# vikramarsid/cadence

Measured on AMD Instinct MI355X. Metric: history events replayed/sec + workflows rebuilt/sec (node), % of HBM roofline, higher is better.
Workload: dtype int64

## Files before the change

### cadence_amd/csrc/replay.hip

```cpp
#include <hip/hip_runtime.h>

#include <cstdio>
#include <cstdlib>
#include <cstring>
#include <type_traits>
#include <vector>

#include "cdr/cdr.h"
#include "ctx.h"

#ifndef CDR_DEPTH
#define CDR_DEPTH 1
#endif
#ifndef CDR_TYPED
#define CDR_TYPED 1
#endif
#ifndef CDR_WPE
#define CDR_WPE 3
#endif
#ifndef CDR_LDS_ACT_MAX
#define CDR_LDS_ACT_MAX 1
#endif
#ifndef CDR_LDS_TIM_MAX
#define CDR_LDS_TIM_MAX 4
// ... 2235 lines not shown
    if (reg0 && carry) {
      launch_reg<CDR_REG0_NA, CDR_REG0_NT, CDR_REG0_NX, CDR_SLICE_REG0, 3, true>(tasks, gr0, sx(3), out_list(Lr0, 3, 1));
      carry_tail(3, gr0, sx(3), true);
    } else if (reg0) {
      typedef RegLds<CDR_REG0_NA, CDR_REG0_NT, CDR_REG0_NX> LY;
      if (cls) {
        typedef ClsLds<CDR_REG0_NA, CDR_REG0_NT, CDR_REG0_NX> LC;
        if (tasks)
          hipLaunchKernelGGL((k_replay_cls<CDR_REG0_NA, CDR_REG0_NT, CDR_REG0_NX, CDR_SLICE_REG0, CDR_WPE_CLS_T, false, true>),
                             gr0, dim3(CDR_SLICE_WIDTH), LC::bytes + CLS_TQ_BYTES, sx(3), with_list(Lr0, 3));
        else
          hipLaunchKernelGGL((k_replay_cls<CDR_REG0_NA, CDR_REG0_NT, CDR_REG0_NX, CDR_SLICE_REG0, CDR_WPE_CLS0>), gr0,
                             dim3(CDR_SLICE_WIDTH), LC::bytes, sx(3), with_list(Lr0, 3));
      }
      if (cls && tasks)
        hipLaunchKernelGGL(k_tasks_merge<CDR_SLICE_REG0>, gr0, dim3(CDR_SLICE_WIDTH), 9 * 65 * 8, sx(3), Lr0);
      if (tasks && !cls)
        hipLaunchKernelGGL((k_replay_reg<CDR_REG0_NA, CDR_REG0_NT, CDR_REG0_NX, CDR_SLICE_REG0, CDR_WPE_REG, false, true>), gr0,
                           dim3(CDR_SLICE_WIDTH), LY::bytes, sx(3), Lr0);
      else if (!cls)
        hipLaunchKernelGGL((k_replay_reg<CDR_REG0_NA, CDR_REG0_NT, CDR_REG0_NX, CDR_SLICE_REG0, 3>), gr0, dim3(CDR_SLICE_WIDTH), LY::bytes, sx(3),
                           Lr0);
    }
        break;
      case 4:
    if (fst && tasks) hipLaunchKernelGGL(k_replay_fast<true>, gf, dim3(CDR_SLICE_WIDTH), FAST_LDS_BYTES + FAST_TBUF_BYTES, sx(4), Lf);
    else if (fst) hipLaunchKernelGGL(k_replay_fast<false>, gf, dim3(CDR_SLICE_WIDTH), FAST_LDS_BYTES, sx(4), Lf);
        break;
      case 5:
    if (reg1 && carry) {
      launch_reg<CDR_REG_NA, CDR_REG_NT, CDR_REG_NX, CDR_SLICE_REG, CDR_WPE_REG, true>(tasks, gr1, sx(5), out_list(Lr1, 5, 1));
      carry_tail(5, gr1, sx(5), true);
    } else if (reg1) {
      typedef RegLds<CDR_REG_NA, CDR_REG_NT, CDR_REG_NX> LY;
      if (cls) {
        typedef ClsLds<CDR_REG_NA, CDR_REG_NT, CDR_REG_NX> LC;
        if (tasks)
          hipLaunchKernelGGL((k_replay_cls<CDR_REG_NA, CDR_REG_NT, CDR_REG_NX, CDR_SLICE_REG, CDR_WPE_CLS_T, false, true>),
                             gr1, dim3(CDR_SLICE_WIDTH), LC::bytes + CLS_TQ_BYTES, sx(5), with_list(Lr1, 5));
        else
          hipLaunchKernelGGL((k_replay_cls<CDR_REG_NA, CDR_REG_NT, CDR_REG_NX, CDR_SLICE_REG, CDR_WPE_CLS>), gr1,
                             dim3(CDR_SLICE_WIDTH), LC::bytes, sx(5), with_list(Lr1, 5));
      }
      if (cls && tasks)
        hipLaunchKernelGGL(k_tasks_merge<CDR_SLICE_REG>, gr1, dim3(CDR_SLICE_WIDTH), 9 * 65 * 8, sx(5), Lr1);
      if (tasks && !cls)
        hipLaunchKernelGGL((k_replay_reg<CDR_REG_NA, CDR_REG_NT, CDR_REG_NX, CDR_SLICE_REG, CDR_WPE_REG, false, true>), gr1,
                           dim3(CDR_SLICE_WIDTH), LY::bytes, sx(5), Lr1);
      else if (!cls)
        hipLaunchKernelGGL((k_replay_reg<CDR_REG_NA, CDR_REG_NT, CDR_REG_NX, CDR_SLICE_REG>), gr1, dim3(CDR_SLICE_WIDTH), LY::bytes, sx(5),
                           Lr1);
    }
        break;
    }
  };
  auto launch_retry = [&](int i) {
    if (!cls || !cls_fb || carry) return;
    switch (i) {
      case 6:
        if (par && !tasks) {
          typedef RegLds<CDR_REG2_NA, CDR_REG_NT, CDR_REG_NX> LY;
          cdr_launch Lp = L;
          Lp.s0 = 0;
          hipLaunchKernelGGL((k_replay_reg<CDR_REG2_NA, CDR_REG_NT, CDR_REG_NX, CDR_SLICE_PAR>), retry_grid(dim3(npar)),
                             dim3(CDR_SLICE_WIDTH), LY::bytes, st, retry_of(with_list(Lp, 6)));
        }
        break;
      case 1:
        if (reg2) {
          typedef RegLds<CDR_REG2_NA, CDR_REG_NT, CDR_REG_NX> LY;
          if (tasks)
            hipLaunchKernelGGL((k_replay_reg<CDR_REG2_NA, CDR_REG_NT, CDR_REG_NX, CDR_SLICE_REG2, CDR_WPE_REG, false, true>),
                               retry_grid(gr2), dim3(CDR_SLICE_WIDTH), LY::bytes, st, retry_of(with_list(Lr2, 1)));
          else
            hipLaunchKernelGGL((k_replay_reg<CDR_REG2_NA, CDR_REG_NT, CDR_REG_NX, CDR_SLICE_REG2>), retry_grid(gr2),
                               dim3(CDR_SLICE_WIDTH), LY::bytes, st, retry_of(with_list(Lr2, 1)));
        }
        break;
      case 3:
        if (reg0) {
          typedef RegLds<CDR_REG0_NA, CDR_REG0_NT, CDR_REG0_NX> LY;
          if (tasks)
            hipLaunchKernelGGL((k_replay_reg<CDR_REG0_NA, CDR_REG0_NT, CDR_REG0_NX, CDR_SLICE_REG0, CDR_WPE_REG, false, true>),
                               retry_grid(gr0), dim3(CDR_SLICE_WIDTH), LY::bytes, st, retry_of(with_list(Lr0, 3)));
          else
            hipLaunchKernelGGL((k_replay_reg<CDR_REG0_NA, CDR_REG0_NT, CDR_REG0_NX, CDR_SLICE_REG0, 3>), retry_grid(gr0),
                               dim3(CDR_SLICE_WIDTH), LY::bytes, st, retry_of(with_list(Lr0, 3)));
        }
        break;
      case 5:
        if (reg1) {
          typedef RegLds<CDR_REG_NA, CDR_REG_NT, CDR_REG_NX> LY;
          if (tasks)
            hipLaunchKernelGGL((k_replay_reg<CDR_REG_NA, CDR_REG_NT, CDR_REG_NX, CDR_SLICE_REG, CDR_WPE_REG, false, true>),
                               retry_grid(gr1), dim3(CDR_SLICE_WIDTH), LY::bytes, st, retry_of(with_list(Lr1, 5)));
          else
            hipLaunchKernelGGL((k_replay_reg<CDR_REG_NA, CDR_REG_NT, CDR_REG_NX, CDR_SLICE_REG>), retry_grid(gr1),
                               dim3(CDR_SLICE_WIDTH), LY::bytes, st, retry_of(with_list(Lr1, 5)));
        }
        break;
    }
  };
  bool issued[cdr_ctx::N_SIDE] = {};
  if (gating) {
    for (int j = 0; j < cdr_ctx::N_SIDE; j++) {
      const int i = order[j] - '0';
      if ((gate && i == 6) || (gate2 && i == 1)) {
        launch_class(i);
        HIPCHK(hipGetLastError());
        issued[i] = true;
      }
    }
    hipStream_t waited[cdr_ctx::N_SIDE + 1];
    int nw = 0;
    for (int q = 0; q < 6; q++) {
      if (!on[q] || q == 1 || (gate && sx(q) == sx(6)) || (gate2 && sx(q) == sx(1))) continue;
      bool dup = false;
      for (int r = 0; r < nw; r++) dup |= waited[r] == sx(q);
      if (dup) continue;
      waited[nw++] = sx(q);
      HIPCHK(hipStreamWaitValue32(sx(q), rws + 15, gate_n, hipStreamWaitValueGte, 0xFFFFFFFFu));
    }
  }
  for (int j = 0; j < cdr_ctx::N_SIDE; j++) {
    const int i = order[j] - '0';
    if (issued[i]) continue;
    launch_class(i);
    HIPCHK(hipGetLastError());
  }
  for (int j = 0; j < cdr_ctx::N_SIDE; j++)
    if (used[j]) {
      HIPCHK(hipEventRecord(c->join[j], c->side[j]));
      HIPCHK(hipStreamWaitEvent(st, c->join[j], 0));
    }
  for (int i : {6, 1, 3, 5}) launch_retry(i);
  HIPCHK(hipGetLastError());
  HIPCHK(hipEventRecord(ring ? c->ring[c->ring_used + 1] : c->ev[1], st));
  if (ring) {
    c->ring_used += 2;
    HIPCHK(hipEventRecord(c->ev[0], st));
    HIPCHK(hipEventRecord(c->ev[1], st));
  }
  const uint32_t fb = (in->n_wfs + 255) / 256;
  const bool all_fast = fst && kinds == 1 && in->n_fast_slices == blocks && gf.x == blocks && !carry && !rws;
  if (fb && !all_fast) hipLaunchKernelGGL(k_tables, dim3(fb), dim3(256), 0, st, *in, *out);
  HIPCHK(hipGetLastError());
  if (fb) hipLaunchKernelGGL(k_finalize, dim3(fb), dim3(256), 0, st, *in, *out);
  HIPCHK(hipGetLastError());
  HIPCHK(hipEventRecord(c->ev[2], st));
  c->timed = true;
  return CDR_API_OK;
}

uint32_t cdr_build_flags(void) {
  uint32_t f = 0;
#ifdef CDR_PAR_PROF
  f |= 1u;
#endif
  if (CDR_PAR_PRIO != 0 || CDR_FDEPTH != 2 || CDR_DEPTH != 1 || CDR_TYPED != 1 || CDR_FAST_DELTA != 1 || CDR_FAST_HINT != 1 ||
      CDR_VHBF != 1 || CDR_VHQUICK != 1 || CDR_CLS_DEPTH != 1 || CDR_CLS_PDEPTH != 4 || CDR_CLS_DEPTH_PAR != 4 ||
      CDR_CLS_PDEPTH_PAR != 16 || CDR_WPE_FAST != 3 || CDR_WPE != 3 || CDR_WPE_CLS != 4 || CDR_WPE_CLS0 != 4 ||
      CDR_WPE_CLS2 != 2 || FAST_CK != 8u || CDR_FAST_TBUF != 5 || CDR_WPE_FAST_TBUF != 2)
    f |= 2u;
  return f;
}

int cdr_last_kernel_ms(cdr_ctx* c, float* replay_ms, float* finalize_ms) {
  if (!c || !c->timed) return CDR_API_EINVAL;
  HIPCHK(hipEventSynchronize(c->ev[2]));
  float a = 0, b = 0;
  HIPCHK(hipEventElapsedTime(&a, c->ev[0], c->ev[1]));
  HIPCHK(hipEventElapsedTime(&b, c->ev[1], c->ev[2]));
  if (replay_ms) *replay_ms = a;
  if (finalize_ms) *finalize_ms = b;
  return CDR_API_OK;
}

int cdr_timing_begin(cdr_ctx* c, uint32_t max_launches) {
  if (!c) return CDR_API_EINVAL;
  HIPCHK(hipSetDevice(c->device));
  while (c->ring.size() < 2ull * max_launches) {
    hipEvent_t e;
    HIPCHK(hipEventCreate(&e));
    c->ring.push_back(e);
  }
  c->ring_used = 0;
  return CDR_API_OK;
}

int cdr_timing_read(cdr_ctx* c, float* ms, uint32_t* n) {
  if (!c || !n) return CDR_API_EINVAL;
  const uint32_t k = c->ring_used / 2;
  for (uint32_t i = 0; i < k && i < *n; i++) {
    HIPCHK(hipEventSynchronize(c->ring[2 * i + 1]));
    HIPCHK(hipEventElapsedTime(&ms[i], c->ring[2 * i], c->ring[2 * i + 1]));
  }
  *n = k < *n ? k : *n;
  c->ring_used = (uint32_t)c->ring.size();
  return CDR_API_OK;
}

}
```

### cadence_amd/csrc/replay_fast.inc

```
#ifndef CDR_WPE_FAST
#define CDR_WPE_FAST 3
#endif
#ifndef CDR_FDEPTH
#define CDR_FDEPTH 2
#endif
constexpr uint32_t FD = CDR_FDEPTH;
#ifndef CDR_VHBF
#define CDR_VHBF 1
#endif
#ifndef CDR_VHQUICK
#define CDR_VHQUICK 1
#endif
#ifndef CDR_FAST_TBUF
#define CDR_FAST_TBUF 5
#endif
#ifndef CDR_TQ_NT
#define CDR_TQ_NT 1
#endif
#ifndef CDR_WPE_FAST_TBUF
#define CDR_WPE_FAST_TBUF 2
#endif
#ifndef CDR_FAST_SADDR
#define CDR_FAST_SADDR 1
#endif
#ifndef CDR_FAST_QROW
#define CDR_FAST_QROW 1
#endif
#ifndef CDR_FAST_DELTA
#define CDR_FAST_DELTA 1
#endif
#ifndef CDR_FAST_HINT
#define CDR_FAST_HINT 1
#endif
#define FAST_LOAD_OPS load_ops<CDR_FAST_DELTA, CDR_NT_FAST, CDR_FAST_HINT != 0>
__device__ __forceinline__ int64_t mov64(int64_t x) {
  int64_t y;
  asm volatile("v_mov_b64 %0, %1" : "=v"(y) : "v"(x));
  return y;
}
__device__ __forceinline__ uint32_t mov32(uint32_t x) {
  uint32_t y;
  asm volatile("v_mov_b32 %0, %1" : "=v"(y) : "v"(x));
  return y;
}
__device__ __forceinline__ uint32_t tf_take(uint32_t t) { return mov32(t); }
__device__ __forceinline__ Ev ev_take(const Ev& q) {
  Ev e;
  e.tf = mov32(q.tf);
  e.h = mov32(q.h);
  e.n = (int32_t)mov32((uint32_t)q.n);
  e.id = mov64(q.id);
  e.ver = mov64(q.ver);
  e.ts = mov64(q.ts);
  e.key = mov64(q.key);
  e.aux = mov64(q.aux);
  return e;
}
#ifndef FAST_CK
#define FAST_CK 8u
#endif
enum : uint32_t {
  ZP_DST_TS = 0, ZP_DSC_TS, ZP_DORIG_TS, ZP_LAST_PROCESSED, ZP_COMPLETION_BATCH,
  ZP_VH_OFF, ZP_RP_OFF, ZP_RUN_RPCAP, ZP_CK0, FAST_COLD = ZP_CK0 + FAST_CK / 2
};
template <class O>
__device__ __forceinline__ GAS cdr_vh_item* fast_out_vh(const O& o) { return gp(o.vh); }
template <class O>
__device__ __forceinline__ GAS cdr_reset_point* fast_out_rp(const O& o) { return gp(o.rp); }
#define VM_DRAIN() __builtin_amdgcn_s_waitcnt(0x0F70)
#define FAST_LDS_BYTES ((CDR_ACT_PLANES + FAST_COLD) * CDR_SLICE_WIDTH * sizeof(uint64_t))
#define FAST_TQ_WORDS (3u * CDR_FAST_TBUF * CDR_SLICE_WIDTH)
#define FAST_TBUF_BYTES (FAST_TQ_WORDS * sizeof(uint64_t))

template <bool TASKS = false>
__global__ __launch_bounds__(CDR_SLICE_WIDTH) __attribute__((amdgpu_waves_per_eu(TASKS && CDR_FAST_TBUF > 0 ? CDR_WPE_FAST_TBUF : CDR_WPE_FAST, 8))) void
k_replay_fast(cdr_launch L) {
  (void)L;
  const uint32_t s = blockIdx.x + KA()->s0;
  const uint32_t lane = threadIdx.x;
  if (s >= KA()->B.ev.n_slices || !KA()->fast) return;
  const uint32_t sflags = __builtin_amdgcn_readfirstlane(KA()->B.ev.slice_flags[s]);
  if (!(sflags & CDR_SLICE_FAST)) return;
  const uint64_t row0_ = KA()->B.ev.slice_row0[s];
  const uint64_t row0 = ((uint64_t)__builtin_amdgcn_readfirstlane((uint32_t)(row0_ >> 32)) << 32) |
                        __builtin_amdgcn_readfirstlane((uint32_t)row0_);
  Slice S;
  S.elems = __builtin_amdgcn_readfirstlane(KA()->B.ev.slice_len[s]) * CDR_SLICE_WIDTH;
  S.r = __builtin_amdgcn_make_buffer_rsrc((void*)(KA()->B.ev.slab + row0 * CDR_ROW_BYTES), (short)0,
                                          (int)(S.elems * CDR_EL_BYTES), 0x00020000);
  S.l4 = lane * 4u;
  const int32_t w = KA()->B.ev.lane_wf[(uint64_t)s * CDR_SLICE_WIDTH + lane];
  if (w < 0 || (KA()->B.skip && KA()->B.skip[w])) return;
#define B_ (KA()->B)
#define O_ (KA()->O)
#define D (gp(B_.wfs)[w])
#define CP (gp(B_.caps)[w])
#define X (gp(O_.exec) + w)
#define vh (gp(O_.vh) + CP.vh_off)
#define rp (gp(O_.rp) + CP.rp_off)
#define sa (gp(O_.sa) + CP.sa_off)
  const uint32_t len = (uint32_t)D.ev_len;
  const bool isVH = D.builder == CDR_BUILDER_NDC;
  const uint32_t EU = B_.empty_uuid;
  const uint32_t vh_cap = CP.vh_cap;
  const LdsSlots<CDR_ACT_PLANES> A{lane};
  const LdsSlots<FAST_COLD> Z{CDR_ACT_PLANES * CDR_SLICE_WIDTH + lane};
  uint32_t hw_act = 0;
  Z.st(0, ZP_DST_TS, 0);
  Z.st(0, ZP_DSC_TS, 0);
  Z.st(0, ZP_DORIG_TS, 0);
  Z.st(0, ZP_LAST_PROCESSED, CDR_EMPTY_EVENT_ID);
  Z.st(0, ZP_COMPLETION_BATCH, 0);
  Z.st(0, ZP_VH_OFF, (int64_t)CP.vh_off);
  Z.st(0, ZP_RP_OFF, (int64_t)CP.rp_off);
  Z.st(0, ZP_RUN_RPCAP, (int64_t)(D.run_id | ((uint64_t)CP.rp_cap << 32)));
#pragma unroll
  for (uint32_t i = 0; i < FAST_CK / 2; i++) Z.st(0, ZP_CK0 + i, 0);
  auto ck_put = [&](uint32_t q, uint32_t c) {
    if (q < FAST_CK) {
      const uint64_t v = (uint64_t)Z.ld(0, ZP_CK0 + q / 2);
      Z.st(0, ZP_CK0 + q / 2,
           (int64_t)((q & 1) ? ((v & 0xFFFFFFFFull) | ((uint64_t)c << 32)) : ((v & ~0xFFFFFFFFull) | c)));
    }
  };
  auto ck_has = [&](uint32_t c) {
    bool x = false;
#pragma unroll
    for (uint32_t i = 0; i < FAST_CK / 2; i++) {
      const uint64_t v = (uint64_t)Z.ld(0, ZP_CK0 + i);
      x |= (uint32_t)v == c || (uint32_t)(v >> 32) == c;
    }
    return x;
  };
#define vh_l (fast_out_vh(O_) + (uint64_t)Z.ld(0, ZP_VH_OFF))
#define rp_l (fast_out_rp(O_) + (uint64_t)Z.ld(0, ZP_RP_OFF))

  uint32_t x_flags = 0, dreq = EU, n_vh = 0, n_rp = 0, n_sa = 0, cks_ok = 0, call_first_k = 0, err_k = 0;
  int32_t x_dt_timeout_value = 0, x_state = CDR_STATE_CREATED, x_close = CDR_CLOSE_NONE, x_signals = 0, dto = 0;
  int32_t err = len == 0 ? CDR_E_HISTORY_EMPTY : CDR_OK;
  int64_t x_next_event = CDR_FIRST_EVENT_ID;
  int64_t dv = CDR_EMPTY_VERSION, dsched = CDR_EMPTY_EVENT_ID, dstart = CDR_EMPTY_EVENT_ID, datt = 0;
  int64_t curv = D.failover_version, vh_last_id = 0, vh_last_ver = 0;
  int64_t call_first_id = 0, prev_id = 0, prev_ver = 0, err_id = 0;
  uint32_t ld = 0;
  const bool want_ld = O_.last_decision != nullptr;
  bool done = len == 0;
  uint32_t n_xt = 0, n_tt = 0, tlist = 0;
  const uint32_t t_xcap = TASKS ? CP.xfer_cap : 0u, t_tcap = TASKS ? CP.ttask_cap : 0u;
  const uint32_t t_dom = TASKS ? D.domain_id : 0u;
  constexpr uint32_t TQ_BASE = (CDR_ACT_PLANES + FAST_COLD) * CDR_SLICE_WIDTH;
  constexpr uint32_t TQ_CAP = CDR_FAST_TBUF * CDR_SLICE_WIDTH;
  uint32_t n_pool = 0;
  const uint64_t t_xoff = TASKS ? (uint64_t)CP.xfer_off : 0u, t_toff = TASKS ? (uint64_t)CP.ttask_off : 0u;
  auto tq_put = [&](bool c, uint32_t kind, uint32_t type, int32_t tt, uint64_t dst, int64_t eid, int64_t v)
      __attribute__((always_inline)) {
    const uint64_t m = __builtin_amdgcn_ballot_w64(c);
    const uint32_t pos = n_pool + __builtin_amdgcn_mbcnt_hi((uint32_t)(m >> 32), __builtin_amdgcn_mbcnt_lo((uint32_t)m, 0u));
    if (c) {
      cdr_lds[TQ_BASE + pos] = (int64_t)(type | ((uint32_t)tt << 8) | (kind << 12) | (dst << 16));
      cdr_lds[TQ_BASE + TQ_CAP + pos] = eid;
      cdr_lds[TQ_BASE + 2u * TQ_CAP + pos] = v;
    }
    n_pool = __builtin_amdgcn_readfirstlane(n_pool + (uint32_t)__builtin_popcountll(m));
  };
  auto task_x = [&](bool c, uint32_t type, int64_t eid, uint32_t dom, uint32_t tl) __attribute__((always_inline)) {
    if constexpr (TASKS) {
      const bool st = c && n_xt < t_xcap;
      if constexpr (CDR_FAST_TBUF > 0) {
        tq_put(st, 0u, type, 0, t_xoff + n_xt, eid, (int64_t)(dom | ((uint64_t)tl << 32)));
      } else if (st) {
        cdr_task t;
        t.type = type;
        t.timeout_type = 0;
        t.event_id = eid;
        t.visibility_ts = 0;
        t.attempt = 0;
        t.domain_id = dom;
        t.task_list = tl;
        t.target_workflow_id = t.target_run_id = t.flags = t._pad = 0;
        t.version = 0;
        gput(gp(O_.transfer) + t_xoff + n_xt, t);
      }
      n_xt += c ? 1u : 0u;
    }
  };
  auto task_t = [&](bool c, uint32_t type, int32_t tt, int64_t eid, int64_t vis) __attribute__((always_inline)) {
// ... 74 lines not shown
  for (uint32_t j = 0; j < FD; j++) T[j] = load_tf<CDR_NT_FAST>(S, el8(j + FD, len, lane));
  const uint32_t srows = S.elems / CDR_SLICE_WIDTH;
  {
    const uint32_t k = 0;
    Ev e = ev_take(Q[0]);
    if (CDR_FAST_HINT) ev_hint(e);
    const uint32_t tn = tf_take(T[0]);
    Q[0] = FAST_LOAD_OPS(S, el8(k + FD, len, lane), tn);
    T[0] = load_tf<CDR_NT_FAST>(S, el8(k + 2 * FD, len, lane));
    call_first_id = SEL(!done, e.id, call_first_id);
    prev_id = SEL(done, prev_id, e.id);
    prev_ver = SEL(done, prev_ver, e.ver);
    if (isVH) {
      const int32_t code =
          (e.id < 0 || (e.ver < 0 && e.ver != CDR_EMPTY_VERSION)) ? CDR_P_VH_ITEM_INVALID
          : (vh_cap == 0)                                            ? CDR_E_BAD_INPUT
                                                                     : CDR_OK;
      curv = SEL(!done, e.ver, curv);
      PFAIL(!done && code != CDR_OK, code);
      n_vh = done ? 0u : 1u;
      vh_last_ver = e.ver;
      vh_last_id = e.id;
    }
    {
      const bool mine = !done;
      const GAS cdr_attr_wf_started* a =
          gp((const cdr_attr_wf_started*)(B_.ev.arena + (uint64_t)(mine ? e.aux : 0)));
      const uint32_t af = a->flags;
      const bool f1 = mine && (af & CDR_SF_HAS_PARENT_DOMAIN) && (af & CDR_SF_PARENT_DOMAIN_MISSING);
      PFAIL(f1, CDR_E_DOMAIN_NOT_FOUND);
      const bool ok = mine && !f1;
      uint32_t nrp = 0, nsa = 0, xf = CDR_XI_STARTED | (isVH ? CDR_XI_VH_BRANCH : CDR_XI_HAS_BRANCH);
      uint32_t h0[32] = {};
      if (ok) {
        const bool retry = (af & CDR_SF_HAS_RETRY) != 0;
        uint64_t lo, hi;
        cdr_uuid(B_.uuid_seed, D.wf_key, CDR_UUID_BRANCH, e.id, &lo, &hi);
        auto q64 = [&](int i, uint64_t v) {
          h0[i] = (uint32_t)v;
          h0[i + 1] = (uint32_t)(v >> 32);
        };
        h0[0] = D.domain_id;
        h0[1] = D.workflow_id;
        h0[2] = D.run_id;
        h0[3] = D.request_id;
        h0[4] = (af & CDR_SF_HAS_PARENT_DOMAIN) ? a->parent_domain_id : 0u;
        h0[5] = (af & CDR_SF_HAS_PARENT_EXEC) ? a->parent_workflow_id : 0u;
        h0[6] = (af & CDR_SF_HAS_PARENT_EXEC) ? a->parent_run_id : 0u;
        h0[7] = a->task_list;
        h0[8] = a->workflow_type;
        h0[9] = a->cron_schedule;
        h0[10] = (af & CDR_SF_HAS_MEMO) ? a->memo : 0u;
        h0[11] = retry ? a->nonretriable : 0u;
        h0[12] = D.run_id;
        h0[13] = (uint32_t)a->exec_timeout_s;
        h0[14] = (uint32_t)a->task_timeout_s;
        h0[15] = (uint32_t)a->attempt;
        q64(16, (uint64_t)((af & CDR_SF_HAS_PARENT_INITIATED) ? a->parent_initiated_id : CDR_EMPTY_EVENT_ID));
        h0[18] = (uint32_t)(retry ? a->retry_initial_s : 0);
        h0[19] = (uint32_t)(retry ? a->retry_max_interval_s : 0);
        q64(20, __builtin_bit_cast(uint64_t, retry ? a->backoff_coefficient : 0.0));
        h0[22] = (uint32_t)(retry ? a->retry_max_attempts : 0);
        h0[23] = (uint32_t)(retry ? a->retry_expiration_s : 0);
        q64(24, (uint64_t)a->expiration_ts);
        q64(26, lo);
        q64(28, hi);
        xf |= a->expiration_ts != 0 ? CDR_XI_HAS_EXPIRATION : 0u;
        xf |= retry ? CDR_XI_HAS_RETRY : 0u;
      }
      {
        constexpr uint32_t RS = 65;
        static_assert(17u * RS * 4u <= CDR_ACT_PLANES * CDR_SLICE_WIDTH * sizeof(uint64_t), "the activity planes");
        uint32_t* const L32 = (uint32_t*)cdr_lds;
        const uint64_t em = __builtin_amdgcn_read_exec();
        const uint32_t rank = __builtin_amdgcn_mbcnt_hi((uint32_t)(em >> 32), __builtin_amdgcn_mbcnt_lo((uint32_t)em, 0u));
        const uint32_t na = (uint32_t)__builtin_popcountll(em);
        typedef unsigned int u32x4 __attribute__((ext_vector_type(4)));
#pragma unroll
        for (uint32_t half = 0; half < 2; half++) {
          __builtin_amdgcn_s_waitcnt(0xC07F);
          __builtin_amdgcn_wave_barrier();
#pragma unroll
          for (uint32_t j = 0; j < 16; j++) L32[j * RS + rank] = h0[16 * half + j];
          L32[16 * RS + rank] = ok ? (uint32_t)w : 0xFFFFFFFFu;
          __builtin_amdgcn_s_waitcnt(0xC07F);
          __builtin_amdgcn_wave_barrier();
          for (uint32_t i = rank; i < 4u * na; i += na) {
            const uint32_t rr = i >> 2, c = i & 3u;
            const uint32_t wr = L32[16 * RS + rr];
            if (wr != 0xFFFFFFFFu) {
              u32x4 v;
              v.x = L32[(4 * c) * RS + rr];
              v.y = L32[(4 * c + 1) * RS + rr];
              v.z = L32[(4 * c + 2) * RS + rr];
              v.w = L32[(4 * c + 3) * RS + rr];
              *((GAS u32x4*)((GAS uint8_t*)(gp(O_.exec) + wr) + 64 * half) + c) = v;
            }
          }
        }
        __builtin_amdgcn_s_waitcnt(0xC07F);
        __builtin_amdgcn_wave_barrier();
      }
      bool f_cap = false;
      if (ok) {
        if (af & CDR_SF_HAS_RESET_POINTS) {
          xf |= CDR_XI_HAS_RESET_POINTS;
          const int64_t expiring = e.ts + (int64_t)D.retention_days * 24ll * 3600ll * NS_PER_S;
          const uint32_t crun = a->continued_run_id, off = a->reset_points_off, cnt = a->reset_points_len;
          const uint32_t cap = CP.rp_cap;
          f_cap |= cnt > cap;
          for (uint32_t q = 0; q < cnt && q < cap; q++) {
            cdr_reset_point p = gget(gp(B_.rps) + (off + q));
            const uint32_t run = (p.flags & CDR_RP_HAS_RUN_ID) ? p.run_id : 0u;
            if (run == crun) {
              p.flags |= CDR_RP_HAS_EXPIRING;
              p.expiring_time_nano = expiring;
            }
            ck_put(nrp, (p.flags & CDR_RP_HAS_CHECKSUM) ? p.binary_checksum : 0u);
            gput(rp + nrp++, p);
          }
        }
        xf |= (af & CDR_SF_HAS_MEMO) ? CDR_XI_HAS_MEMO : 0u;
        if (af & CDR_SF_HAS_SEARCH_ATTR) {
          const uint32_t off = a->search_attr_off, cnt = a->search_attr_len, cap = CP.sa_cap;
          f_cap |= cnt > cap;
          nsa = cnt < cap ? cnt : cap;
          for (uint32_t q = 0; q < nsa; q++) {
            const cdr_kv kv = gget(gp(B_.kvs) + (off + q));
            uint32_t rank = 0;
            for (uint32_t j = 0; j < nsa; j++) {
              const uint32_t kj = gp(B_.kvs)[off + j].key;
              rank += (kj < kv.key || (kj == kv.key && j < q)) ? 1u : 0u;
            }
            gput(sa + rank, kv);
          }
          xf |= nsa ? CDR_XI_HAS_SEARCH_ATTR : 0u;
        }
      }
      PFAIL(f_cap, CDR_E_BAD_INPUT);
      n_rp = SEL(ok, nrp, n_rp);
      n_sa = SEL(ok, nsa, n_sa);
      x_flags = SEL(ok, xf, x_flags);
      x_dt_timeout_value = SEL(ok, a->task_timeout_s, x_dt_timeout_value);
      if constexpr (TASKS) {
        tlist = ok ? a->task_list : 0u;
        const int64_t backoff = ok ? (int64_t)a->first_decision_backoff_s * NS_PER_S : 0;
        task_t(ok && backoff != 0, CDR_TT_WORKFLOW_BACKOFF, (af & CDR_SF_CRON_INITIATOR) ? 1 : 0, 0, e.ts + backoff);
        task_t(ok, CDR_TT_WORKFLOW_TIMEOUT, 0, 0, e.ts + (int64_t)(ok ? a->exec_timeout_s : 0) * NS_PER_S + backoff);
        task_x(ok, CDR_TT_RECORD_STARTED, 0, 0, 0);
      }
    }
    VM_DRAIN();
  }
#if CDR_FAST_SADDR
  const uint32_t lane8 = lane * 8u;
  auto el8q = [&](uint32_t kk) {
    return __builtin_amdgcn_readfirstlane((kk < srows ? kk : srows - 1u) * CDR_ROW_BYTES) + lane8;
  };
#else
  auto el8q = [&](uint32_t kk) { return el8(kk, len, lane); };
#endif
  auto step = [&](const uint32_t k, Ev& q, uint32_t& t) __attribute__((always_inline)) {
    Ev e = ev_take(q);
    const uint32_t tn = tf_take(t);
    q = FAST_LOAD_OPS(S, el8q(k + FD), tn);
    t = load_tf<CDR_NT_FAST>(S, el8q(k + 2 * FD));
    const uint32_t type = e.tf & 0xFFu;
#if CDR_FAST_QROW
    const int64_t qid = (int64_t)((uint64_t)prev_id + 1u);
    const bool qlane = !done && k < len && (e.tf & CDR_SEF_ID_NEXT) && (e.tf & CDR_SEF_VER_SAME) &&
                       (!isVH || (n_vh != 0 && qid >= 0));
    if (__builtin_amdgcn_ballot_w64(!qlane) == 0) {
      e.id = qid;
      e.ver = prev_ver;
      const bool bf = (e.tf & CDR_SEF_BATCH_FIRST) != 0;
      x_next_event = SEL(bf, qid, x_next_event);
      call_first_id = SEL(bf, qid, call_first_id);
      call_first_k = SEL(bf, k, call_first_k);
      ld = SEL(bf, 0u, ld);
      prev_id = qid;
      vh_last_id = SEL(isVH, qid, vh_last_id);
    } else
#endif
    {
    e.id = (e.tf & CDR_SEF_ID_NEXT) ? (int64_t)((uint64_t)prev_id + 1u) : e.id;
    e.ver = (e.tf & CDR_SEF_VER_SAME) ? prev_ver : e.ver;
    done |= k >= len;
    const bool bf = !done && ((e.tf & CDR_SEF_BATCH_FIRST) || k == 0);
    x_next_event = SEL(bf && k > 0, prev_id + 1, x_next_event);
    call_first_id = SEL(bf, e.id, call_first_id);
    call_first_k = SEL(bf, k, call_first_k);
    ld = SEL(bf, 0u, ld);
    prev_id = SEL(done, prev_id, e.id);
    prev_ver = SEL(done, prev_ver, e.ver);
    if (isVH) {
      curv = SEL(!done && (x_state == CDR_STATE_CREATED || x_state == CDR_STATE_RUNNING), e.ver, curv);
#if CDR_VHQUICK
      const bool quick = done || (n_vh != 0 && (e.tf & CDR_SEF_ID_NEXT) && (e.tf & CDR_SEF_VER_SAME) && e.id >= 0);
      if (__builtin_amdgcn_ballot_w64(!quick) == 0) {
        vh_last_id = SEL(done, vh_last_id, e.id);
      } else
#endif
      {
#if CDR_VHBF
      const bool has = n_vh != 0;
      const bool newitem = !has | (e.ver > vh_last_ver);
      const bool b_inv = (e.id < 0) | ((e.ver < 0) & (e.ver != CDR_EMPTY_VERSION));
      const bool b_ver = has & (e.ver < vh_last_ver);
      const bool b_id = has & (e.id <= vh_last_id);
      const bool b_cap = newitem & (n_vh >= vh_cap);
      int32_t code = b_cap ? (int32_t)CDR_E_BAD_INPUT : (int32_t)CDR_OK;
      code = b_id ? (int32_t)CDR_E_VH_LOWER_EVENT_ID : code;
      code = b_ver ? (int32_t)CDR_E_VH_LOWER_VERSION : code;
      code = b_inv ? (int32_t)CDR_P_VH_ITEM_INVALID : code;
#else
      const bool newitem = n_vh == 0 || e.ver > vh_last_ver;
      const int32_t code = (e.id < 0 || (e.ver < 0 && e.ver != CDR_EMPTY_VERSION)) ? CDR_P_VH_ITEM_INVALID
                           : (n_vh != 0 && e.ver < vh_last_ver)                     ? CDR_E_VH_LOWER_VERSION
                           : (n_vh != 0 && e.id <= vh_last_id)                      ? CDR_E_VH_LOWER_EVENT_ID
                           : (newitem && n_vh >= vh_cap)                            ? CDR_E_BAD_INPUT
                                                                                    : CDR_OK;
#endif
      PFAIL(!done && code != CDR_OK, code);
      const bool add = !done && newitem;
      const bool put = add && n_vh != 0;
      if (put) gput(vh_l + (n_vh - 1), cdr_vh_item{vh_last_id, vh_last_ver});
      if (__builtin_amdgcn_ballot_w64(put)) VM_DRAIN();
      n_vh += add ? 1u : 0u;
      vh_last_ver = SEL(add, e.ver, vh_last_ver);
      vh_last_id = SEL(done, vh_last_id, e.id);
      }
    }
    }
    if (CDR_FAST_HINT) ev_hint(e);
    for (uint64_t pend = __builtin_amdgcn_ballot_w64(!done); pend;) {
      uint32_t ut = __builtin_amdgcn_readlane(type, __builtin_ctzll(pend));
      asm volatile("" : "+s"(ut));
      const bool mine = !done && type == ut;
      pend &= ~__builtin_amdgcn_ballot_w64(mine);
      switch (ut) {
        case CDR_EV_DT_SCHEDULED:
          dv = SEL(mine, e.ver, dv);
          dsched = SEL(mine, e.id, dsched);
          dstart = SEL(mine, CDR_EMPTY_EVENT_ID, dstart);
          dreq = SEL(mine, EU, dreq);
          dto = SEL(mine, e.n, dto);
          datt = SEL(mine, e.aux, datt);
          ld = SEL(mine, ld_make(CDR_LD_SCHEDULED, k), ld);
          if (mine) {
            Z.st(0, ZP_DSC_TS, e.ts);
            Z.st(0, ZP_DST_TS, 0);
            Z.st(0, ZP_DORIG_TS, e.ts);
          }
          task_x(mine, CDR_TT_DECISION, e.id, t_dom, tlist);
          break;
        case CDR_EV_DT_STARTED: {
          const bool f = mine && e.key != dsched;
          PFAIL(f, CDR_E_DECISION_NOT_FOUND);
          const bool ok = mine && !f;
          x_state = SEL(ok && x_state == CDR_STATE_CREATED, (int32_t)CDR_STATE_RUNNING, x_state);
          dv = SEL(ok, e.ver, dv);
          dstart = SEL(ok, e.id, dstart);
          dreq = SEL(ok, e.h, dreq);
          datt = SEL(ok, (int64_t)0, datt);
          ld = SEL(ok, ld_make(CDR_LD_STARTED, k), ld);
          if (ok) Z.st(0, ZP_DST_TS, e.ts);
          task_t(ok, CDR_TT_DECISION_TIMEOUT, CDR_TIMEOUT_START_TO_CLOSE, e.key, e.ts + (int64_t)dto * NS_PER_S);
          break;
        }
        case CDR_EV_DT_COMPLETED: {
          FLD_CAPTURE(mine);
          dv = SEL(mine, CDR_EMPTY_VERSION, dv);
          dsched = SEL(mine, CDR_EMPTY_EVENT_ID, dsched);
          dstart = SEL(mine, CDR_EMPTY_EVENT_ID, dstart);
          dreq = SEL(mine, EU, dreq);
          dto = SEL(mine, 0, dto);
          datt = SEL(mine, (int64_t)0, datt);
          if (mine) {
            Z.st(0, ZP_DST_TS, 0);
            Z.st(0, ZP_DSC_TS, 0);
            Z.st(0, ZP_LAST_PROCESSED, e.aux);
          }
          const uint32_t cks = e.h;
          const bool chk = mine && cks != 0 && cks != cks_ok;
          if (__builtin_amdgcn_ballot_w64(chk)) {
            bool exists = chk && ck_has(cks);
            const bool deep = chk && !exists && n_rp > FAST_CK;
            if (__builtin_amdgcn_ballot_w64(deep)) {
              for (uint32_t q = FAST_CK; deep && q < n_rp; q++) {
                const cdr_reset_point p = gget(rp_l + q);
                exists |= ((p.flags & CDR_RP_HAS_CHECKSUM) ? p.binary_checksum : 0u) == cks;
              }
            }
            const uint64_t rc = (uint64_t)Z.ld(0, ZP_RUN_RPCAP);
            const bool app = chk && !exists;
            const bool f = app && n_rp >= (uint32_t)(rc >> 32);
            PFAIL(f, CDR_E_BAD_INPUT);
            const bool put = app && !f;
            if (put) {
              cdr_reset_point p;
              p.binary_checksum = cks;
              p.run_id = (uint32_t)rc;
              p.first_decision_completed_id = e.id;
              p.created_time_nano = B_.now_ns;
              p.expiring_time_nano = 0;
              p.flags = CDR_RP_HAS_CHECKSUM | CDR_RP_HAS_RUN_ID | CDR_RP_HAS_FIRST_DC_ID | CDR_RP_HAS_CREATED |
                        CDR_RP_HAS_RESETTABLE | CDR_RP_RESETTABLE;
              p._pad = 0;
              gput(rp_l + n_rp, p);
              ck_put(n_rp, cks);
            }
            if (__builtin_amdgcn_ballot_w64(put)) VM_DRAIN();
            n_rp += put ? 1u : 0u;
            x_flags |= put ? CDR_XI_HAS_RESET_POINTS : 0u;
            cks_ok = SEL(chk && !f, cks, cks_ok);
          }
          break;
        }
        case CDR_EV_DT_TIMED_OUT:
        case CDR_EV_DT_FAILED: {
          FLD_CAPTURE(mine);
          const bool inc = ut == CDR_EV_DT_FAILED || e.n != CDR_TIMEOUT_SCHEDULE_TO_START;
          const int64_t now = B_.now_ns;
          const int64_t na = inc ? datt + 1 : 0;
          const bool tr = na != 0;
          dv = SEL(mine, tr ? (isVH ? curv : CDR_EMPTY_VERSION) : CDR_EMPTY_VERSION, dv);
          dsched = SEL(mine, tr ? x_next_event : CDR_EMPTY_EVENT_ID, dsched);
          dstart = SEL(mine, CDR_EMPTY_EVENT_ID, dstart);
          dreq = SEL(mine, EU, dreq);
          dto = SEL(mine, tr ? x_dt_timeout_value : 0, dto);
          if (mine) {
            Z.st(0, ZP_DST_TS, 0);
            Z.st(0, ZP_DORIG_TS, 0);
            Z.st(0, ZP_DSC_TS, (tr || inc) ? now : (int64_t)0);
          }
          task_x(mine && tr, CDR_TT_DECISION, x_next_event, t_dom, tlist);
          datt = SEL(mine, na, datt);
          ld = SEL(mine && tr, ld_make(CDR_LD_TRANSIENT, k), ld);
          break;
        }
        case CDR_EV_AT_SCHEDULED: {
          const bool f = mine && hw_act != 0 && A.ld(0, AP_SID) != DEAD_KEY;
          PFAIL(f, CDR_E_BAD_INPUT);
          const bool ok = mine && !f;
          hw_act = SEL(ok, 1u, hw_act);
          if (ok) {
            const uint32_t aid = (uint32_t)e.key;
            const int32_t s2c = (int32_t)e.h, s2s = e.n;
            const int64_t t_s2c = e.ts + (int64_t)s2c * NS_PER_S, t_s2s = e.ts + (int64_t)s2s * NS_PER_S;
            const uint32_t bit = t_s2s < t_s2c ? CDR_TTS_SCHEDULE_TO_START : CDR_TTS_SCHEDULE_TO_CLOSE;
            A.st(0, AP_SID, e.id);
            A.st(0, AP_TS2C, t_s2c);
            A.st(0, AP_TALT, t_s2s);
            A.st(0, AP_THB, T_NONE);
            A.st(0, AP_META, (int64_t)(aid | META_FLAG(AF_AIDMAP) | ((uint64_t)bit << META_TTS_SHIFT)));
            A.st(0, AP_VER, e.ver);
            A.st(0, AP_STARTED_ID, CDR_EMPTY_EVENT_ID);
            A.st(0, AP_STARTED_TIME, 0);
            A.st(0, AP_CANCEL_ID, CDR_EMPTY_EVENT_ID);
            A.st(0, AP_ROWS, (int64_t)(k | ((uint64_t)call_first_k << 32)));
            A.st(0, AP_STC_HB, (int64_t)(((uint64_t)e.key >> 32) | ((uint64_t)e.aux & 0xFFFFFFFF00000000ull)));
            A.st(0, AP_REQ, 0);
          }
          if constexpr (TASKS) {
            task_x(ok, CDR_TT_ACTIVITY, e.id, t_dom, tlist);
            const int64_t t_s2c = e.ts + (int64_t)(int32_t)e.h * NS_PER_S, t_s2s = e.ts + (int64_t)e.n * NS_PER_S;
            const bool s2s = t_s2s < t_s2c;
            task_t(ok, CDR_TT_ACTIVITY_TIMEOUT, s2s ? CDR_TIMEOUT_SCHEDULE_TO_START : CDR_TIMEOUT_SCHEDULE_TO_CLOSE, e.id,
                   s2s ? t_s2s : t_s2c);
          }
          break;
        }
        case CDR_EV_AT_STARTED: {
          const bool f = mine && !(hw_act != 0 && A.ld(0, AP_SID) == e.key);
          PFAIL(f, CDR_P_ACTIVITY_STARTED_NIL);
          bool t_made = false;
          int32_t t_tt = 0;
          int64_t t_vis = 0;
          if (mine && !f) {
            const uint64_t th = (uint64_t)A.ld(0, AP_STC_HB);
            const int32_t stc = (int32_t)(uint32_t)th, hb = (int32_t)(uint32_t)(th >> 32);
            const uint64_t m = (uint64_t)A.ld(0, AP_META) | META_FLAG(AF_STARTED);
            const int64_t t0 = A.ld(0, AP_TS2C);
            const int64_t ta = e.ts + (int64_t)stc * NS_PER_S;
            const int64_t tb = hb > 0 ? e.ts + (int64_t)hb * NS_PER_S : T_NONE;
            const int64_t t1 = ta < t0 ? ta : t0;
            const uint32_t bit =
                tb < t1 ? CDR_TTS_HEARTBEAT : (ta < t0 ? CDR_TTS_START_TO_CLOSE : CDR_TTS_SCHEDULE_TO_CLOSE);
            A.st(0, AP_VER, e.ver);
            A.st(0, AP_STARTED_ID, e.id);
            A.st(0, AP_REQ, (int64_t)e.h);
            A.st(0, AP_STARTED_TIME, e.ts);
            A.st(0, AP_TALT, ta);
            A.st(0, AP_THB, tb);
            A.st(0, AP_META, (int64_t)(m | ((uint64_t)bit << META_TTS_SHIFT)));
            if constexpr (TASKS) {
              t_made = !(m & ((uint64_t)bit << META_TTS_SHIFT));
              t_tt = (int32_t)__builtin_ctz(bit);
              t_vis = tb < t1 ? tb : t1;
            }
          }
          task_t(t_made, CDR_TT_ACTIVITY_TIMEOUT, t_tt, e.key, t_vis);
          break;
        }
        case CDR_EV_AT_COMPLETED:
        case CDR_EV_AT_FAILED:
        case CDR_EV_AT_TIMED_OUT:
        case CDR_EV_AT_CANCELED: {
          const bool live = hw_act != 0 && A.ld(0, AP_SID) == e.key;
          PFAIL(mine && !live, CDR_E_ACTIVITY_NOT_FOUND);
          const bool ok = mine && live;
          PFAIL(ok && !((uint64_t)A.ld(0, AP_META) & META_FLAG(AF_AIDMAP)), CDR_E_ACTIVITY_ID_NOT_FOUND);
          if (ok) A.st(0, AP_SID, DEAD_KEY);
          break;
        }
        case CDR_EV_AT_CANCEL_REQUESTED: {
          const uint64_t m = (uint64_t)A.ld(0, AP_META);
          const bool hit = hw_act != 0 && A.ld(0, AP_SID) != DEAD_KEY && (uint32_t)m == (uint32_t)e.key &&
                           (m & META_FLAG(AF_AIDMAP));
          PFAIL(mine && !hit, CDR_E_MISSING_ACTIVITY_INFO);
          if (mine && hit) {
            A.st(0, AP_VER, e.ver);
            A.st(0, AP_META, (int64_t)(m | META_FLAG(AF_CANCEL)));
            A.st(0, AP_CANCEL_ID, e.id);
          }
          break;
        }
        case CDR_EV_AT_REQ_CANCEL_FAILED:
        case CDR_EV_CANCEL_TIMER_FAILED:
        case CDR_EV_MARKER_RECORDED:
          break;
        case CDR_EV_WF_SIGNALED:
          x_signals += mine ? 1 : 0;
          break;
        case CDR_EV_WF_CANCEL_REQUESTED:
          x_flags |= mine ? CDR_XI_CANCEL_REQUESTED : 0u;
          break;
        case CDR_EV_WF_COMPLETED:
        case CDR_EV_WF_FAILED:
        case CDR_EV_WF_TIMED_OUT:
        case CDR_EV_WF_CANCELED:
        case CDR_EV_WF_TERMINATED: {
          const int cs = ut == CDR_EV_WF_COMPLETED   ? CDR_CLOSE_COMPLETED
                         : ut == CDR_EV_WF_FAILED    ? CDR_CLOSE_FAILED
                         : ut == CDR_EV_WF_TIMED_OUT ? CDR_CLOSE_TIMED_OUT
                         : ut == CDR_EV_WF_CANCELED  ? CDR_CLOSE_CANCELED
                                                     : CDR_CLOSE_TERMINATED;
          const bool f = mine && !transition_ok(x_state, x_close, CDR_STATE_COMPLETED, cs);
          PFAIL(f, CDR_E_INVALID_STATE_TRANSITION);
          const bool ok = mine && !f;
          x_state = SEL(ok, (int32_t)CDR_STATE_COMPLETED, x_state);
          x_close = SEL(ok, (int32_t)cs, x_close);
          if (ok) Z.st(0, ZP_COMPLETION_BATCH, call_first_id);
          task_x(ok, CDR_TT_CLOSE_EXECUTION, 0, 0, 0);
          task_t(ok, CDR_TT_DELETE_HISTORY, 0, 0, e.ts + (int64_t)D.retention_days * 86400ll * NS_PER_S);
          break;
        }
        default:
          PFAIL(mine, CDR_E_BAD_INPUT);
          break;
      }
    }
    if constexpr (TASKS) {
      if constexpr (CDR_FAST_TBUF > 0) {
        if (n_pool + 2u * CDR_SLICE_WIDTH > TQ_CAP) {
          tq_flush();
          VM_DRAIN();
        }
      } else {
        VM_DRAIN();
      }
    }
  };
  static_assert(FD >= 1 && FD <= 3, "CDR_FDEPTH");
  for (uint32_t k = 1; k < srows; k += FD) {
    if (__builtin_amdgcn_ballot_w64(!done) == 0) break;
    step(k, Q[1 % FD], T[1 % FD]);
    if (FD > 1) step(k + 1, Q[2 % FD], T[2 % FD]);
    if (FD > 2) step(k + 2, Q[3 % FD], T[3 % FD]);
  }
#undef PFAIL
#undef SEL
#undef FLD_CAPTURE
  if constexpr (TASKS && CDR_FAST_TBUF > 0) tq_flush();
  if (len > 0 && err == CDR_OK) x_next_event = prev_id + 1;
  if (err == CDR_OK && D.parent < 0 && D.expected_next_event_id != 0 && x_next_event != D.expected_next_event_id) {
    err = CDR_E_REBUILD_NEXT_EVENT_ID;
    err_id = prev_id;
    err_k = len;
  }
  if (TASKS && err == CDR_OK && (n_xt > t_xcap || n_tt > t_tcap)) {
    err = CDR_E_BAD_INPUT;
    err_id = prev_id;
    err_k = len;
  }
  const bool ok = err == CDR_OK;
  const bool act_live = ok && hw_act != 0 && A.ld(0, AP_SID) != DEAD_KEY;
  cdr_wf_result r;
  r.code = err;
  r.flags = D.parent >= 0 ? CDR_RF_IS_NEWRUN : 0u;
  r.fail_event_id = err_id;
  r.fail_index = err_k;
  r.n_activity = act_live ? 1u : 0u;
  r.n_timer = r.n_child = r.n_cancel = r.n_signal = 0;
  r.n_vh = ok ? n_vh : 0u;
  r.n_reset_points = ok ? n_rp : 0u;
  r.n_search_attr = ok ? n_sa : 0u;
  if constexpr (TASKS) {
    gp(O_.n_tasks)[2 * (uint64_t)w] = ok ? n_xt : 0u;
    gp(O_.n_tasks)[2 * (uint64_t)w + 1] = ok ? n_tt : 0u;
  }
  const bool ld_on = ok && want_ld && !(ld & LD_CAPTURED);
  const cdr_last_decision ldr =
      ld_rec(ld, dv, dsched, dstart, dreq, dto, datt, Z.ld(0, ZP_DSC_TS), Z.ld(0, ZP_DST_TS), Z.ld(0, ZP_DORIG_TS));
  cdr_activity_info o{};
  if (act_live) {
    const uint64_t rows = (uint64_t)A.ld(0, AP_ROWS);
    const uint32_t o_s = el8((uint32_t)rows, len, lane), o_b = el8((uint32_t)(rows >> 32), len, lane);
    const int64_t sched_ts = bld64(S.r, o_s, S.col(CDR_COL_TIMESTAMP));
    const uint32_t arec = (uint32_t)bld64(S.r, o_s, S.col(CDR_COL_AUX));
    const GAS cdr_attr_at_scheduled* a = gp((const cdr_attr_at_scheduled*)(B_.ev.arena + arec));
    const uint64_t m = (uint64_t)A.ld(0, AP_META);
    const bool retry = (a->flags & CDR_AF_HAS_RETRY) != 0;
    const int32_t s2c = a->s2c_s, xs = a->retry_expiration_s;
    o.version = A.ld(0, AP_VER);
    o.schedule_id = A.ld(0, AP_SID);
    o.scheduled_event_batch_id = bld64(S.r, o_b, S.col(CDR_COL_EVENT_ID));
    o.scheduled_time = sched_ts;
    o.started_id = A.ld(0, AP_STARTED_ID);
    o.started_time = A.ld(0, AP_STARTED_TIME);
    o.last_heartbeat_time = A.ld(0, AP_STARTED_TIME);
    o.expiration_time = sched_ts + (int64_t)((retry && xs > s2c) ? xs : s2c) * NS_PER_S;
    o.cancel_request_id = A.ld(0, AP_CANCEL_ID);
    o.activity_id = (uint32_t)m;
    o.request_id = (uint32_t)A.ld(0, AP_REQ);
    o.task_list = a->task_list;
    o.nonretriable = retry ? a->nonretriable : 0u;
    o.s2s = a->s2s_s;
    o.s2c = s2c;
    o.stc = a->stc_s;
    o.hb = a->hb_s;
    o.timer_task_status = (int32_t)((m >> META_TTS_SHIFT) & 0xFFu);
    o.attempt = 0;
    o.initial_interval = retry ? a->retry_initial_s : 0;
    o.maximum_interval = retry ? a->retry_max_interval_s : 0;
    o.maximum_attempts = retry ? a->retry_max_attempts : 0;
    o.flags = (retry ? CDR_AI_HAS_RETRY : 0u) | ((m & META_FLAG(AF_CANCEL)) ? CDR_AI_CANCEL_REQUESTED : 0u) |
              ((m & META_FLAG(AF_STARTED)) ? CDR_AI_STARTED_TIME_SET : 0u);
    o.backoff_coefficient = retry ? a->backoff_coefficient : 0.0;
  }
  uint32_t hv[32] = {};
  {
    auto p64 = [&](int i, int64_t v) {
      hv[i] = (uint32_t)v;
      hv[i + 1] = (uint32_t)((uint64_t)v >> 32);
    };
    hv[0] = dreq;
    hv[1] = x_flags;
    p64(2, Z.ld(0, ZP_COMPLETION_BATCH));
    hv[4] = (uint32_t)x_state;
    hv[5] = (uint32_t)x_close;
    p64(6, call_first_id);
    p64(8, bld64(S.r, el8(len - 1, len, lane), S.col(CDR_COL_TASK_ID)));
    p64(10, x_next_event);
    p64(12, Z.ld(0, ZP_LAST_PROCESSED));
    hv[14] = (uint32_t)x_signals;
    hv[15] = (uint32_t)dto;
    p64(16, dv);
    p64(18, dsched);
    p64(20, dstart);
    p64(22, datt);
    p64(24, Z.ld(0, ZP_DST_TS));
    p64(26, Z.ld(0, ZP_DSC_TS));
    p64(28, Z.ld(0, ZP_DORIG_TS));
    hv[30] = n_rp;
    hv[31] = n_sa;
  }
  const bool vh_on = ok && n_vh;
  const cdr_vh_item vi{vh_last_id, vh_last_ver};
  GAS cdr_vh_item* const vh_dst = vh_on ? vh + (n_vh - 1) : nullptr;
  GAS cdr_activity_info* const act_dst = act_live ? gp(O_.act) + CP.act_off : nullptr;
  coop_put<7>(gp(O_.result) + w, r, true, 0);
  coop_put<10>(gp(O_.last_decision) + w, ldr, ld_on, 0);
  coop_put<9>(act_dst, o, act_live, 0);
  coop_put<2>(vh_dst, vi, vh_on, 0);
  {
    constexpr uint32_t RS = 65;
    static_assert(33u * RS * 4u <= FAST_LDS_BYTES, "the transpose fits the planes it reuses");
    uint32_t* const L32 = (uint32_t*)cdr_lds;
    const uint64_t em = __builtin_amdgcn_read_exec();
    const uint32_t rank = __builtin_amdgcn_mbcnt_hi((uint32_t)(em >> 32), __builtin_amdgcn_mbcnt_lo((uint32_t)em, 0u));
    const uint32_t na = (uint32_t)__builtin_popcountll(em);
    __builtin_amdgcn_s_waitcnt(0xC07F);
    __builtin_amdgcn_wave_barrier();
#pragma unroll
    for (uint32_t j = 0; j < 32; j++) L32[j * RS + rank] = hv[j];
    L32[32 * RS + rank] = ok ? (uint32_t)w : 0xFFFFFFFFu;
    __builtin_amdgcn_s_waitcnt(0xC07F);
    __builtin_amdgcn_wave_barrier();
    typedef unsigned int u32x4 __attribute__((ext_vector_type(4)));
    for (uint32_t i = rank; i < 8u * na; i += na) {
      const uint32_t rr = i >> 3, c = i & 7u;
      const uint32_t wr = L32[32 * RS + rr];
      if (wr != 0xFFFFFFFFu) {
        u32x4 v;
        v.x = L32[(4 * c) * RS + rr];
        v.y = L32[(4 * c + 1) * RS + rr];
        v.z = L32[(4 * c + 2) * RS + rr];
        v.w = L32[(4 * c + 3) * RS + rr];
        *((GAS u32x4*)((GAS uint8_t*)(gp(O_.exec) + wr) + 128) + c) = v;
      }
    }
  }
#undef D
#undef CP
#undef X
#undef vh
#undef rp
#undef vh_l
#undef rp_l
#undef sa
#undef B_
#undef O_
}
```

Before: 141.6 billion.

## Add wave-uniform fast replay loop that uses scalar type-flags to skip column loads

Adds a specialised step path for rows where every lane in the wavefront has the same event type-flags. It reads the flags once with readfirstlane and branches on them uniformly, skipping the per-type readlane/ballot dispatch loop and issuing column buffer loads only for the fields that row actually needs. The loop falls back to the original divergent step once any lane's flags differ or the end of the slice is near. This raises code size and register pressure, and it helps only when workflows in a wave share the same event sequence.

```diff
diff --git a/cadence_amd/csrc/replay.hip b/cadence_amd/csrc/replay.hip
--- a/cadence_amd/csrc/replay.hip
+++ b/cadence_amd/csrc/replay.hip
@@ -2411,6 +2411,8 @@
   return CDR_API_OK;
 }
 
+#define CDR_STR_(...) #__VA_ARGS__
+#define CDR_STR(...) CDR_STR_(__VA_ARGS__)
 uint32_t cdr_build_flags(void) {
   uint32_t f = 0;
 #ifdef CDR_PAR_PROF
@@ -2419,7 +2421,9 @@
   if (CDR_PAR_PRIO != 0 || CDR_FDEPTH != 2 || CDR_DEPTH != 1 || CDR_TYPED != 1 || CDR_FAST_DELTA != 1 || CDR_FAST_HINT != 1 ||
       CDR_VHBF != 1 || CDR_VHQUICK != 1 || CDR_CLS_DEPTH != 1 || CDR_CLS_PDEPTH != 4 || CDR_CLS_DEPTH_PAR != 4 ||
       CDR_CLS_PDEPTH_PAR != 16 || CDR_WPE_FAST != 3 || CDR_WPE != 3 || CDR_WPE_CLS != 4 || CDR_WPE_CLS0 != 4 ||
-      CDR_WPE_CLS2 != 2 || FAST_CK != 8u || CDR_FAST_TBUF != 5 || CDR_WPE_FAST_TBUF != 2)
+      CDR_WPE_CLS2 != 2 || FAST_CK != 8u || CDR_FAST_TBUF != 5 || CDR_WPE_FAST_TBUF != 2 || CDR_FAST_UNI != 1 || CDR_FAST_UNI_SKIP != 1 ||
+      CDR_NT_FAST != 2 || CDR_NT_CLS != 0 || CDR_FAST_SADDR != 1 || CDR_FAST_QROW != 1 || CDR_CLS_TBUF != 3 ||
+      CDR_MERGE_D2 != 0 || sizeof(CDR_STR(CDR_MERGE_ATTR)) != 1 )
     f |= 2u;
   return f;
 }
diff --git a/cadence_amd/csrc/replay_fast.inc b/cadence_amd/csrc/replay_fast.inc
--- a/cadence_amd/csrc/replay_fast.inc
+++ b/cadence_amd/csrc/replay_fast.inc
@@ -32,6 +32,14 @@
 #ifndef CDR_FAST_HINT
 #define CDR_FAST_HINT 1
 #endif
+#ifndef CDR_FAST_UNI
+#define CDR_FAST_UNI 1
+#endif
+#ifndef CDR_FAST_UNI_SKIP
+#define CDR_FAST_UNI_SKIP 1
+#endif
+struct fast_uni_no { static constexpr bool value = false; };
+struct fast_uni_yes { static constexpr bool value = true; };
 #define FAST_LOAD_OPS load_ops<CDR_FAST_DELTA, CDR_NT_FAST, CDR_FAST_HINT != 0>
 __device__ __forceinline__ int64_t mov64(int64_t x) {
   int64_t y;
@@ -412,37 +420,22 @@
     }
     VM_DRAIN();
   }
+  const uint32_t lane8 = lane * 8u;
 #if CDR_FAST_SADDR
-  const uint32_t lane8 = lane * 8u;
   auto el8q = [&](uint32_t kk) {
     return __builtin_amdgcn_readfirstlane((kk < srows ? kk : srows - 1u) * CDR_ROW_BYTES) + lane8;
   };
 #else
   auto el8q = [&](uint32_t kk) { return el8(kk, len, lane); };
 #endif
-  auto step = [&](const uint32_t k, Ev& q, uint32_t& t) __attribute__((always_inline)) {
-    Ev e = ev_take(q);
-    const uint32_t tn = tf_take(t);
-    q = FAST_LOAD_OPS(S, el8q(k + FD), tn);
-    t = load_tf<CDR_NT_FAST>(S, el8q(k + 2 * FD));
-    const uint32_t type = e.tf & 0xFFu;
-#if CDR_FAST_QROW
-    const int64_t qid = (int64_t)((uint64_t)prev_id + 1u);
-    const bool qlane = !done && k < len && (e.tf & CDR_SEF_ID_NEXT) && (e.tf & CDR_SEF_VER_SAME) &&
-                       (!isVH || (n_vh != 0 && qid >= 0));
-    if (__builtin_amdgcn_ballot_w64(!qlane) == 0) {
-      e.id = qid;
-      e.ver = prev_ver;
-      const bool bf = (e.tf & CDR_SEF_BATCH_FIRST) != 0;
-      x_next_event = SEL(bf, qid, x_next_event);
-      call_first_id = SEL(bf, qid, call_first_id);
-      call_first_k = SEL(bf, k, call_first_k);
-      ld = SEL(bf, 0u, ld);
-      prev_id = qid;
-      vh_last_id = SEL(isVH, qid, vh_last_id);
-    } else
-#endif
-    {
+#if CDR_FAST_UNI
+#if !CDR_FAST_UNI_SKIP
+  const rsrc_t r_none = __builtin_amdgcn_make_buffer_rsrc((void*)(KA()->B.ev.slab + row0 * CDR_ROW_BYTES), (short)0, 0, 0x00020000);
+  auto rs = [&](bool need) { return need ? S.r : r_none; };
+#endif
+  auto rowq = [&](uint32_t kk) { return __builtin_amdgcn_readfirstlane((kk < srows ? kk : srows - 1u) * CDR_ROW_BYTES); };
+#endif
+  auto general_row = [&](Ev& e, const uint32_t k) __attribute__((always_inline)) {
     e.id = (e.tf & CDR_SEF_ID_NEXT) ? (int64_t)((uint64_t)prev_id + 1u) : e.id;
     e.ver = (e.tf & CDR_SEF_VER_SAME) ? prev_ver : e.ver;
     done |= k >= len;
@@ -491,13 +484,107 @@
       vh_last_id = SEL(done, vh_last_id, e.id);
       }
     }
+  };
+  auto step = [&](auto uni_, const uint32_t k, Ev& q, uint32_t& t, const uint32_t stf, const uint32_t stn)
+      __attribute__((always_inline)) {
+    constexpr bool UNI = decltype(uni_)::value;
+    Ev e;
+    if constexpr (UNI) {
+#if CDR_FAST_UNI
+      e.tf = stf;
+      e.h = mov32(q.h);
+      e.n = (int32_t)mov32((uint32_t)q.n);
+      e.id = mov64(q.id);
+      e.ver = mov64(q.ver);
+      e.ts = mov64(q.ts);
+      e.key = mov64(q.key);
+      e.aux = mov64(q.aux);
+      t = bld32<CDR_NT_FAST>(S.r, S.l4 + S.col(CDR_COL_TYPE_FLAGS), rowq(k + 2 * FD));
+      const uint32_t so = rowq(k + FD);
+      const uint32_t kbn = CDR_FAST_HINT ? (stn & CDR_SEF_KEY_BACK) : 0u, ain = CDR_FAST_HINT ? (stn & CDR_SEF_AUX_IMPL) : 0u;
+      q.tf = stn;
+#if CDR_FAST_UNI_SKIP
+#define UNI_LD64(need, c_) ((need) ? bld64<CDR_NT_FAST>(S.r, lane8 + S.col(c_), so) : (int64_t)0)
+#define UNI_LD32(need, c_) ((need) ? bld32<CDR_NT_FAST>(S.r, S.l4 + S.col(c_), so) : 0u)
+#else
+#define UNI_LD64(need, c_) bld64<CDR_NT_FAST>(rs(need), lane8 + S.col(c_), so)
+#define UNI_LD32(need, c_) bld32<CDR_NT_FAST>(rs(need), S.l4 + S.col(c_), so)
+#endif
+      q.id = UNI_LD64(!(CDR_FAST_DELTA && (stn & CDR_SEF_ID_NEXT)), CDR_COL_EVENT_ID);
+      q.ver = UNI_LD64(!(CDR_FAST_DELTA && (stn & CDR_SEF_VER_SAME)), CDR_COL_VERSION);
+      q.ts = UNI_LD64((stn & CDR_SEF_NEED_TS) != 0, CDR_COL_TIMESTAMP);
+      q.key = UNI_LD64((stn & CDR_SEF_NEED_KEY) && !kbn, CDR_COL_KEY);
+      q.aux = UNI_LD64((stn & CDR_SEF_NEED_AUX) && !ain, CDR_COL_AUX);
+      q.h = UNI_LD32((stn & CDR_SEF_NEED_H) != 0, CDR_COL_H);
+      q.n = (int32_t)UNI_LD32((stn & CDR_SEF_NEED_N) != 0, CDR_COL_N);
+#undef UNI_LD64
+#undef UNI_LD32
+#endif
+    } else {
+      e = ev_take(q);
+      const uint32_t tn = tf_take(t);
+      q = FAST_LOAD_OPS(S, el8q(k + FD), tn);
+      t = load_tf<CDR_NT_FAST>(S, el8q(k + 2 * FD));
+    }
+    const uint32_t type = e.tf & 0xFFu;
+    if constexpr (UNI) {
+      const int64_t qid = (int64_t)((uint64_t)prev_id + 1u);
+      const bool qlane = !done && (!isVH || (n_vh != 0 && qid >= 0));
+      if (CDR_FAST_QROW && (stf & CDR_SEF_ID_NEXT) && (stf & CDR_SEF_VER_SAME) && __builtin_amdgcn_ballot_w64(!qlane) == 0) {
+        e.id = qid;
+        e.ver = prev_ver;
+        if (stf & CDR_SEF_BATCH_FIRST) {
+          x_next_event = qid;
+          call_first_id = qid;
+          call_first_k = k;
+          ld = 0u;
+        }
+        prev_id = qid;
+        vh_last_id = SEL(isVH, qid, vh_last_id);
+      } else {
+        general_row(e, k);
+      }
+      if (CDR_FAST_HINT) {
+        const uint32_t kb = (stf & CDR_SEF_KEY_BACK) >> CDR_SEF_KEY_BACK_SHIFT;
+        const uint32_t ai = (stf & CDR_SEF_AUX_IMPL) >> CDR_SEF_AUX_IMPL_SHIFT;
+        if (kb) e.key = (int64_t)((uint64_t)e.id - kb);
+        if (ai && ai != CDR_SEF_AUX_ZERO) e.aux = (int64_t)((uint64_t)e.id - ai);
+      }
+    } else {
+#if CDR_FAST_QROW
+    const int64_t qid = (int64_t)((uint64_t)prev_id + 1u);
+    const bool qlane = !done && k < len && (e.tf & CDR_SEF_ID_NEXT) && (e.tf & CDR_SEF_VER_SAME) &&
+                       (!isVH || (n_vh != 0 && qid >= 0));
+    if (__builtin_amdgcn_ballot_w64(!qlane) == 0) {
+      e.id = qid;
+      e.ver = prev_ver;
+      const bool bf = (e.tf & CDR_SEF_BATCH_FIRST) != 0;
+      x_next_event = SEL(bf, qid, x_next_event);
+      call_first_id = SEL(bf, qid, call_first_id);
+      call_first_k = SEL(bf, k, call_first_k);
+      ld = SEL(bf, 0u, ld);
+      prev_id = qid;
+      vh_last_id = SEL(isVH, qid, vh_last_id);
+    } else
+#endif
+    {
+      general_row(e, k);
     }
     if (CDR_FAST_HINT) ev_hint(e);
-    for (uint64_t pend = __builtin_amdgcn_ballot_w64(!done); pend;) {
-      uint32_t ut = __builtin_amdgcn_readlane(type, __builtin_ctzll(pend));
-      asm volatile("" : "+s"(ut));
-      const bool mine = !done && type == ut;
-      pend &= ~__builtin_amdgcn_ballot_w64(mine);
+    }
+    for (uint64_t pend = UNI ? 1u : __builtin_amdgcn_ballot_w64(!done); pend;) {
+      uint32_t ut;
+      bool mine;
+      if constexpr (UNI) {
+        ut = type;
+        mine = !done;
+        pend = 0;
+      } else {
+        ut = __builtin_amdgcn_readlane(type, __builtin_ctzll(pend));
+        asm volatile("" : "+s"(ut));
+        mine = !done && type == ut;
+        pend &= ~__builtin_amdgcn_ballot_w64(mine);
+      }
       switch (ut) {
         case CDR_EV_DT_SCHEDULED:
           dv = SEL(mine, e.ver, dv);
@@ -733,11 +820,28 @@
     }
   };
   static_assert(FD >= 1 && FD <= 3, "CDR_FDEPTH");
-  for (uint32_t k = 1; k < srows; k += FD) {
+  uint32_t k = 1;
+#if CDR_FAST_UNI
+  for (; k + FD <= srows; k += FD) {
+    uint32_t stf[FD], stn[FD];
+    bool nu = k + FD > len;
+#pragma unroll
+    for (uint32_t j = 0; j < FD; j++) {
+      stf[j] = __builtin_amdgcn_readfirstlane(Q[(1 + j) % FD].tf);
+      stn[j] = __builtin_amdgcn_readfirstlane(T[(1 + j) % FD]);
+      nu |= Q[(1 + j) % FD].tf != stf[j] || T[(1 + j) % FD] != stn[j];
+    }
+    if (__builtin_amdgcn_ballot_w64(nu) != 0 || __builtin_amdgcn_ballot_w64(!done) == 0) break;
+    step(fast_uni_yes{}, k, Q[1 % FD], T[1 % FD], stf[0], stn[0]);
+    if (FD > 1) step(fast_uni_yes{}, k + 1, Q[2 % FD], T[2 % FD], stf[1 % FD], stn[1 % FD]);
+    if (FD > 2) step(fast_uni_yes{}, k + 2, Q[3 % FD], T[3 % FD], stf[2 % FD], stn[2 % FD]);
+  }
+#endif
+  for (; k < srows; k += FD) {
     if (__builtin_amdgcn_ballot_w64(!done) == 0) break;
-    step(k, Q[1 % FD], T[1 % FD]);
-    if (FD > 1) step(k + 1, Q[2 % FD], T[2 % FD]);
-    if (FD > 2) step(k + 2, Q[3 % FD], T[3 % FD]);
+    step(fast_uni_no{}, k, Q[1 % FD], T[1 % FD], 0u, 0u);
+    if (FD > 1) step(fast_uni_no{}, k + 1, Q[2 % FD], T[2 % FD], 0u, 0u);
+    if (FD > 2) step(fast_uni_no{}, k + 2, Q[3 % FD], T[3 % FD], 0u, 0u);
   }
 #undef PFAIL
 #undef SEL
```

New measurement: 153.2 billion (median of 6 runs). +8.2%, better.
